# Luka140/paig_reproduction

Measured on AMD Instinct MI355X. Metric: video-seqs/sec (train step) spring_color B=100 @ 1/2/4/8 MI355X, higher is better.
Workload: dtype fp32; 1 GPU; spring_color PhysicsNet train step (get_batch gather+fwd+loss+bwd+allreduce+RMSprop), B=100/rank, 32x32x3, seq_len 50 (4 in / 6 pred / 40 extrap); global_batch=100, seq_len=50, parallelism=dp1, conv_math=split, split_graph=False, optimizer_in_graph=True, byte_targets=True, dataset_seqs=800

## Files before the change

### paig_reproduction_amd/csrc/conv_bwd.hip

```cpp
#include "split_common.h"

#include <stdlib.h>

#ifndef PAIG_BWD_MINW
#define PAIG_BWD_MINW 0
#endif
#ifndef PAIG_BWD_UPS2
#define PAIG_BWD_UPS2 1
#endif
#ifndef PAIG_BWD_TPX_C10
#define PAIG_BWD_TPX_C10 0
#define PAIG_BWD_MINW_C10 0
#endif
#ifndef PAIG_BWD_PSD_EVEN_C10
#define PAIG_BWD_PSD_EVEN_C10 0
#endif
#ifndef PAIG_BWD_AUXP
#define PAIG_BWD_AUXP 1
#endif

#ifdef PAIG_BWD_STAMPS
__device__ unsigned long long paig_bwd_stamps[4096][4][13];
#define PAIG_BSTAMP(k)                                      \
  do {                                                      \
// ... 9 lines not shown

namespace {

constexpr int sbwd_lds(int CIN, int COUT, int H, int W, bool UPS, int PM, int tpx) {
  const int FPT = H * W <= tpx ? tpx / (H * W) : 1, RT = H * W <= tpx ? H : rows_fit(H, W, tpx);
  const bool pe = PAIG_BWD_PSD_EVEN_C10 && UPS && CIN == 16 && COUT == 16 && H == 32;
  const int ROWS = RT + 2, ROWSD = ROWS + (UPS ? 2 : 0), CCD = rup(COUT, 8) / 8,
            PSD = CCD % 2 == 0 && !pe ? CCD + 1 : CCD;
  const int RPD = W == 8 ? to_mod16((W + 2) * PSD, 8) : (W + 2) * PSD;
  const int IMGD = (FPT * ROWSD * RPD + 2) * 8, WIMG = ceil_div(9 * CCD, 4) * ceil_div(CIN, 16) * 64 * 8;
  const int XIMG = rup(CIN, 4) / 4 * rup(FPT * ROWS * (W + 4) * 4 + 80, 128) * 2 * (PM == 2 ? 1 : 2);
  const int UPB = UPS ? CIN * (rup(FPT * (RT + 2) * W, 64) + 4) * 4 : 0;
  const int XREG = XIMG > UPB ? XIMG : UPB;
  return (IMGD + WIMG) * 2 * (PM == 2 ? 1 : 2) + XREG + (UPS ? up_window_floats(CIN, FPT, RT, W) * 4 : 0);
}
constexpr int sbwd_tpx(int CIN, int COUT, int H, int W, bool UPS, int PM) {
  if (PAIG_BWD_TPX_C10 && UPS && CIN == 16 && COUT == 16 && H == 32) return PAIG_BWD_TPX_C10;
  for (int pass = 0; pass < 2; ++pass)
    for (int t = 256; t >= 64; t /= 2) {
      const int rt = H * W <= t ? H : rows_fit(H, W, t);
      if (UPS && (rt % 2 != 0 || H * W < t)) continue;
      if (sbwd_lds(CIN, COUT, H, W, UPS, PM, t) <= (pass == 0 ? LDS_MAX / 2 : LDS_MAX)) return t;
    }
  return 64;
}

constexpr int sbwd_minw(int CIN, int COUT, int H, int PM, bool PF) {
  if (PAIG_BWD_MINW_C10 && CIN == 16 && COUT == 16 && H == 32) return PAIG_BWD_MINW_C10;
  if (CIN == 8 && COUT == 8 && H == 32) return PF || PAIG_BWD_AUXP == 2 ? 3 : 4;
  if (PM == 2 && CIN == 8 && COUT == 16 && H == 16) return 3;
  if (PM == 2 && CIN == 24 && COUT == 8 && H == 32) return 3;
  if (CIN == 8 && COUT == 8 && H == 36) return PF ? 2 : 3;
  if (CIN == 8 && COUT == 16 && H == 18) return PM == 2 ? 4 : 3;
  if (CIN == 16 && COUT == 16 && H == 18) return PF ? 2 : 3;
  return 2;
}

constexpr bool sbwd_auxp(int CIN, int COUT, int H, int PM, bool UPS, bool PF) {
  if (PAIG_BWD_AUXP == 2) return true;
  if (CIN == 8 && COUT == 8 && (H == 32 || H == 36) && !PF) return false;
  if (CIN == 24 && COUT == 8 && (H == 36 || PM == 2)) return false;
  if (UPS && H == 36) return false;
  if (PM == 0) return !(PF && CIN == 16 && COUT == 16 && H == 16);
  return !((UPS && CIN == 32 && H == 16) || (CIN == 8 && COUT == 16 && H == 16));
}

template <int CIN, int COUT, int H, int W, int KS, bool UPS, int PM, bool PF = false>
struct SBwdCfg {
  static constexpr int KK = KS * KS, PADL = KS / 2;
  static constexpr int NIMG = PM == 2 ? 1 : 2;
  static constexpr int TPX = sbwd_tpx(CIN, COUT, H, W, UPS, PM);
  static constexpr int FPT = H * W <= TPX ? TPX / (H * W) : 1;
  static constexpr int RT = H * W <= TPX ? H : rows_fit(H, W, TPX);
  static constexpr int TPXV = FPT * RT * W;
  static constexpr int ROWS = RT + KS - 1;
  static constexpr int EXT = UPS ? 1 : 0;
  static constexpr int RTD = RT + 2 * EXT, ROWSD = ROWS + 2 * EXT;
  static constexpr int TPXD = FPT * RTD * W;
  static constexpr int CCD = rup(COUT, 8) / 8;
  static constexpr bool PSDE = PAIG_BWD_PSD_EVEN_C10 && UPS && CIN == 16 && COUT == 16 && H == 32;
  static constexpr int PSD = CCD % 2 == 0 && !PSDE ? CCD + 1 : CCD;
  static constexpr int TWPX = W + 2 * PADL;
  static constexpr int RPD = W == 8 ? to_mod16(TWPX * PSD, 8) : TWPX * PSD;
  static constexpr int ZSLOT = FPT * ROWSD * RPD;
  static constexpr int IMGD = (ZSLOT + 2) * 8;
  static constexpr int KC = KK * CCD, NS = ceil_div(KC, 4);
  static constexpr int NTD = ceil_div(CIN, 16);
  static constexpr int NMT = ceil_div(TPXD, 16), MW = ceil_div(NMT, 4);
  static constexpr int WIMG = NS * NTD * 64 * 8;
  static constexpr int CQ = rup(CIN, 4) / 4, NQ = KK * CQ, NTX = ceil_div(NQ, 4);
  static constexpr int OFFX = PADL > 0 ? 2 : 0, TWX = W + 2 * OFFX;
  static constexpr int XPL = rup(FPT * ROWS * TWX * 4 + 80, 128);
  static constexpr int XIMG = CQ * XPL;
  static constexpr int MT = ceil_div(COUT, 16), NTW = ceil_div(NTX, 4);
  static constexpr bool BAL = !(PM == 2 && (CIN == 24 || (UPS && CIN == 32) || H == 36 || H == 18)) && !(H == 36 && !UPS && !PF);
  static constexpr int NTF = BAL ? NTX / 4 : ceil_div(NTX, 4), NTR = BAL ? NTX % 4 : 0;
  static constexpr int KB = ceil_div(TPXV, 32);
  static constexpr int NCOL = CIN * KK, SLAB = COUT * NCOL + COUT;
  static constexpr int UPX = W % 2 == 0 ? 2 : 1, W2 = W / UPX;
  static constexpr int NID = FPT * ROWSD * W2 * CCD, NLD = ceil_div(NID, 256);
  static constexpr int NIX = FPT * ROWS * W2 * CQ, NLX = ceil_div(NIX, 256);
  static constexpr int UPW = up_window_floats(CIN, FPT, RT, W);
  static constexpr int UPB = UPS ? CIN * (rup(FPT * (RT + 2) * W, 64) + 4) * 4 : 0;
  static constexpr int XREG = XIMG * 2 * NIMG > UPB ? XIMG * 2 * NIMG : UPB;
  static constexpr int LDS = (IMGD + WIMG) * 2 * NIMG + XREG + (UPS ? UPW * 4 : 0);
  static constexpr bool VEC4 = W % 4 == 0;
  static constexpr bool XPIPE = !UPS && NLX * 8 <= 32;
  static constexpr int LDSB = LDS_MAX / (LDS > (NLD * 256 * 8 + 256) * 4 ? LDS : (NLD * 256 * 8 + 256) * 4);
  static constexpr int MW0 = PAIG_BWD_MINW > 0 ? PAIG_BWD_MINW : sbwd_minw(CIN, COUT, H, PM, PF);
  static constexpr int MINW = MW0 < LDSB ? MW0 : LDSB;
  static_assert(H % RT == 0, "RT divides H");
  static_assert(KS == 3, "3x3 layers (the 1x1 heads are fused elsewhere)");
  static_assert(!UPS || (FPT == 1 && RT % 2 == 0 && W % 2 == 0), "fused upsample: whole even row blocks of one frame");
  static_assert(!PF || (!UPS && UPX == 2 && COUT % 8 == 0 && H % 2 == 0), "pool fold: even widths, 8-channel chunks");
  static constexpr int UPP = rup(TPXD, 64) + 4;
  static_assert(!UPS || CIN * UPP * 4 <= XREG, "fused upsample: dX tile does not fit the X region");
  static constexpr int WSU = W / 2, IKU = WSU % 4 == 0 ? 4 : (WSU % 2 == 0 ? 2 : 1), WQU = WSU / IKU;
  static constexpr int NOU = UPS ? CIN * (RT / 2) * WQU : 0, NOI = NOU > 0 ? ceil_div(NOU, 256) : 1;
  static constexpr bool AUXP =
      PAIG_BWD_AUXP && (UPS || (VEC4 && MW * NTD <= 8)) && sbwd_auxp(CIN, COUT, H, PM, UPS, PF);
};

template <int CIN, int COUT, int H, int W, int KS, bool UPS, int PM, bool PF>
__global__ void __launch_bounds__(256, (SBwdCfg<CIN, COUT, H, W, KS, UPS, PM, PF>::MINW))
conv_bwd_split_k(FView x, FView dy, FViewW dx, FView aux, const float* __restrict__ w, int flags,
                 float* __restrict__ slab, int F, int ntiles, XMax xm, const s16x8* __restrict__ wp, FView dpool,
                 const unsigned char* __restrict__ pcode, long long pcode_fs) {
  using C = SBwdCfg<CIN, COUT, H, W, KS, UPS, PM, PF>;
  constexpr int KK = C::KK, PADL = C::PADL, RT = C::RT, FPT = C::FPT, ROWS = C::ROWS, TPXV = C::TPXV;
  constexpr int EXT = C::EXT, RTD = C::RTD, ROWSD = C::ROWSD, TPXD = C::TPXD;
  constexpr int CCD = C::CCD, PSD = C::PSD, RPD = C::RPD, KC = C::KC, NS = C::NS, NTD = C::NTD, MW = C::MW;
  constexpr int CQ = C::CQ, NQ = C::NQ, NTX = C::NTX, OFFX = C::OFFX, TWX = C::TWX, XPL = C::XPL;
  constexpr int MT = C::MT, NTF = C::NTF, NTR = C::NTR, KB = C::KB, NCOL = C::NCOL, UPX = C::UPX, W2 = C::W2;
  constexpr int NF1 = NTF > 0 ? NTF : 1, NR1 = NTR > 0 ? NTR : 1;
  constexpr int NID = C::NID, NLD = C::NLD, NIX = C::NIX, NLX = C::NLX;
  constexpr long long HW = (long long)H * W;
  constexpr long long XPLANE = UPS ? (long long)(H / 2) * (W / 2) : HW;
  constexpr int NRB = H / RT;
  extern __shared__ __attribute__((aligned(16))) short lds16[];
  short* Dh = lds16;
  short* Dl = Dh + (C::NIMG == 2 ? C::IMGD : 0);
  short* Wh = lds16 + C::NIMG * C::IMGD;
  short* Wl = Wh + (C::NIMG == 2 ? C::WIMG : 0);
  short* Xh = lds16 + C::NIMG * (C::IMGD + C::WIMG);
  short* Xl = Xh + (C::NIMG == 2 ? C::XIMG : 0);
// ... 122 lines not shown
  for (int t = 0; t < NTR; ++t) coltr[t] = colt_of(NTF * 4 + t);
  auto dslot = [&](int j) {
    if (TPXV % 32 != 0 && j >= TPXV) return C::ZSLOT;
    const int fi = j / (RT * W), rem = j % (RT * W);
    return (fi * ROWSD + rem / W + PADL + EXT) * RPD + (rem % W + PADL) * PSD;
  };
  auto xpos = [&](int j) {
    if (TPXV % 32 != 0 && j >= TPXV) j = 0;
    const int fi = j / (RT * W), rem = j % (RT * W);
    return ((fi * ROWS + rem / W) * TWX + rem % W + (OFFX - PADL)) * 4;
  };

  f32x4 accw[MT][NF1], accr[MT][NR1];
#pragma unroll
  for (int m = 0; m < MT; ++m) {
#pragma unroll
    for (int j = 0; j < NF1; ++j) accw[m][j] = f32x4{0.f, 0.f, 0.f, 0.f};
#pragma unroll
    for (int t = 0; t < NR1; ++t) accr[m][t] = f32x4{0.f, 0.f, 0.f, 0.f};
  }
  float bacc[NLD][8];
#pragma unroll
  for (int l = 0; l < NLD; ++l)
#pragma unroll
    for (int c = 0; c < 8; ++c) bacc[l][c] = 0.f;

  float2 pd[NLD][8];
  float2 px[C::XPIPE ? NLX : 1][4];
  float dpv[PF ? NLD : 1][8];
  uint2 pcv[PF ? NLD : 1];
  constexpr int HP = H / 2, WP = W / 2;
  using UP = UpStage<UPS ? CIN : 1, H, W, FPT, RT>;
  UP up;
  auto load_d = [&](int t) {
    const int f0 = (t / NRB) * FPT, y0 = (t % NRB) * RT;
    const float* fb = dy.frame(f0 < F ? f0 : 0);
#pragma unroll
    for (int l = 0; l < NLD; ++l) {
      const int i = tid + l * 256;
      const int xp = UPX * (i % W2), r = (i / W2) % ROWSD, cc = (i / (W2 * ROWSD)) % CCD, fi = i / (W2 * ROWSD * CCD);
      const int gy = y0 + r - PADL - EXT;
#ifdef PAIG_BWD_NOLOAD
      const bool ok = false;
#else
      const bool ok = i < NID && f0 + fi < F && gy >= 0 && gy < H;
#endif
      const int off = fi * (int)dy.fs + cc * 8 * (int)HW + gy * W + xp;
      static_assert(8 * HW <= 8 * 4096, "paig_zero_planes covers the unit");
      const float* base = ok ? fb + off : paig_zero_planes;
#pragma unroll
      for (int c = 0; c < 8; ++c) {
        const float* q = COUT % 8 == 0 || cc * 8 + c < COUT ? base + c * (int)HW : paig_zeros;
        pd[l][c] = UPX == 2 ? *reinterpret_cast<const float2*>(q) : make_float2(*q, 0.f);
      }
      if constexpr (PF) {
        const int pw = (gy >> 1) * WP + (xp >> 1);
        const float* pb = ok ? dpool.frame(f0) + fi * (int)dpool.fs + cc * 8 * (HP * WP) + pw : paig_zero_planes;
#pragma unroll
        for (int c = 0; c < 8; ++c) dpv[l][c] = pb[c * (HP * WP)];
        const unsigned char* cb = ok ? pcode + (long long)(f0 + fi) * pcode_fs + ((long long)cc * HP * WP + pw) * 8
                                     : reinterpret_cast<const unsigned char*>(paig_zeros);
        pcv[l] = *reinterpret_cast<const uint2*>(cb);
      }
    }
  };
  auto fold = [&](int t) {
    const int y0 = (t % NRB) * RT;
#pragma unroll
    for (int l = 0; l < NLD; ++l) {
      const int i = tid + l * 256;
      const int r = (i / W2) % ROWSD;
      const int pr = ((y0 + r - PADL - EXT) & 1) * 2;
#pragma unroll
      for (int c = 0; c < 8; ++c) {
        const unsigned b = ((c < 4 ? pcv[l].x : pcv[l].y) >> (8 * (c & 3))) & 255u;
        const int am = (int)(b >> 4) & 3;
        const float vx = pd[l][c].x + (am == pr ? dpv[l][c] : 0.f);
        const float vy = pd[l][c].y + (am == pr + 1 ? dpv[l][c] : 0.f);
        pd[l][c].x = (b >> pr) & 1u ? vx : 0.f;
        pd[l][c].y = (b >> (pr + 1)) & 1u ? vy : 0.f;
      }
    }
  };
  auto load_x = [&](int t, int i, float2* v) {
    const int f0 = (t / NRB) * FPT, y0 = (t % NRB) * RT;
    const int xp = UPX * (i % W2), r = (i / W2) % ROWS, cq = (i / (W2 * ROWS)) % CQ, fi = i / (W2 * ROWS * CQ);
    const int gy = y0 + r - PADL;
    const bool ok = i < NIX && f0 + fi < F && gy >= 0 && gy < H;
    const float* fb = x.frame(f0 < F ? f0 : 0);
    const int off = fi * (int)x.fs + cq * 4 * (int)XPLANE + gy * W + xp;
    const float* base = ok ? fb + off : paig_zero_planes;
#pragma unroll
    for (int c = 0; c < 4; ++c) {
      const float* q = CIN % 4 == 0 || cq * 4 + c < CIN ? base + c * (int)XPLANE : paig_zeros;
      v[c] = UPX == 2 ? *reinterpret_cast<const float2*>(q) : make_float2(*q, 0.f);
    }
  };
  auto issue = [&](int t) {
    load_d(t);
    if constexpr (UPS) {
      up.issue(x, F, (t / NRB) * FPT, (t % NRB) * RT, tid);
    } else if constexpr (C::XPIPE) {
#pragma unroll
      for (int l = 0; l < NLX; ++l) load_x(t, tid + l * 256, px[l]);
    }
  };
  auto put_d = [&](int i, const float2* v) {
    const int xp = UPX * (i % W2), r = (i / W2) % ROWSD, cc = (i / (W2 * ROWSD)) % CCD, fi = i / (W2 * ROWSD * CCD);
    const int o = ((fi * ROWSD + r) * RPD + (xp + PADL) * PSD + cc) * 8;
    s16x8 h0, l0, h1, l1;
    if constexpr (PM == 0) {
      pf32x2 sv[8];
#pragma unroll
      for (int c = 0; c < 8; ++c) sv[c] = pf32x2{v[c].x, v[c].y} * dsc;
      u32x4 a0, b0, a1, b1;
#pragma unroll
      for (int k = 0; k < 4; ++k) {
        { const HiLo q_ = split_pk(sv[2 * k].x, sv[2 * k + 1].x); a0[k] = q_.h; b0[k] = q_.l; }
        { const HiLo q_ = split_pk(sv[2 * k].y, sv[2 * k + 1].y); a1[k] = q_.h; b1[k] = q_.l; }
      }
      h0 = __builtin_bit_cast(s16x8, a0);
      l0 = __builtin_bit_cast(s16x8, b0);
      h1 = __builtin_bit_cast(s16x8, a1);
      l1 = __builtin_bit_cast(s16x8, b1);
    } else {
      float rm = 0.f;
#pragma unroll
      for (int c = 0; c < 8; ++c) {
        short h, lo;
        split<PM>(v[c].x, h, lo, rm);
        h0[c] = h;
        l0[c] = lo;
        split<PM>(v[c].y, h, lo, rm);
        h1[c] = h;
        l1[c] = lo;
      }
    }
    *reinterpret_cast<s16x8*>(Dh + o) = h0;
    if (PM != 2) *reinterpret_cast<s16x8*>(Dl + o) = l0;
    if constexpr (UPX == 2) {
      *reinterpret_cast<s16x8*>(Dh + o + PSD * 8) = h1;
      if (PM != 2) *reinterpret_cast<s16x8*>(Dl + o + PSD * 8) = l1;
    }
  };
  auto put_x = [&](int i, const float2* v) {
    const int xp = UPX * (i % W2), r = (i / W2) % ROWS, cq = (i / (W2 * ROWS)) % CQ, fi = i / (W2 * ROWS * CQ);
    const int o = xplane(cq) + ((fi * ROWS + r) * TWX + xp + OFFX) * 4;
    s16x8 hv, lv;
    if constexpr (PM == 0) {
      pf32x2 sv[4];
#pragma unroll
      for (int c = 0; c < 4; ++c) {
        sv[c] = pf32x2{v[c].x, v[c].y} * xsc;
        rmax = amax2(rmax, sv[c].x, sv[c].y);
      }
      u32x4 a, b;
      { const HiLo q_ = split_pk(sv[0].x, sv[1].x); a[0] = q_.h; b[0] = q_.l; }
      { const HiLo q_ = split_pk(sv[2].x, sv[3].x); a[1] = q_.h; b[1] = q_.l; }
      { const HiLo q_ = split_pk(sv[0].y, sv[1].y); a[2] = q_.h; b[2] = q_.l; }
      { const HiLo q_ = split_pk(sv[2].y, sv[3].y); a[3] = q_.h; b[3] = q_.l; }
      hv = __builtin_bit_cast(s16x8, a);
      lv = __builtin_bit_cast(s16x8, b);
    } else {
#pragma unroll
      for (int c = 0; c < 4; ++c) {
        short h, lo;
        split<PM>(v[c].x, h, lo, rmax);
        hv[c] = h;
        lv[c] = lo;
        split<PM>(v[c].y, h, lo, rmax);
        hv[4 + c] = h;
        lv[4 + c] = lo;
      }
    }
    if constexpr (UPX == 2) {
      *reinterpret_cast<s16x8*>(Xh + o) = hv;
      if (PM != 2) *reinterpret_cast<s16x8*>(Xl + o) = lv;
    } else {
      *reinterpret_cast<s16x4*>(Xh + o) = s16x4{hv[0], hv[1], hv[2], hv[3]};
      if (PM != 2) *reinterpret_cast<s16x4*>(Xl + o) = s16x4{lv[0], lv[1], lv[2], lv[3]};
    }
  };
  auto tile_max = [&]() {
    float m = 0.f;
#pragma unroll
    for (int l = 0; l < NLD; ++l)
#pragma unroll
      for (int c = 0; c < 8; ++c) m = amax2(m, pd[l][c].x, pd[l][c].y);
    m = wave_max_u(m);
    if (lane == 0) smax[wv] = m;
  };
  auto commit = [&](int t) {
    if constexpr (PM == 0 && PAIG_SCALE_MODE < 2) {
      const int te = f16_scale_exp(fmaxf(fmaxf(smax[0], smax[1]), fmaxf(smax[2], smax[3])));
      const int td = te < ecd + 64 ? te : ecd + 64;
      if (td != ecd) {
#pragma unroll
        for (int m = 0; m < MT; ++m)
#pragma unroll
          for (int r = 0; r < 4; ++r) {
#pragma unroll
            for (int j = 0; j < NF1; ++j) accw[m][j][r] = __builtin_amdgcn_ldexpf(accw[m][j][r], td - ecd);
#pragma unroll
            for (int t = 0; t < NR1; ++t) accr[m][t][r] = __builtin_amdgcn_ldexpf(accr[m][t][r], td - ecd);
          }
        ecd = td;
        dsc = __builtin_amdgcn_ldexpf(1.f, ecd);
      }
    }
    const int f0 = (t / NRB) * FPT;
#pragma unroll
    for (int l = 0; l < NLD; ++l) {
      const int i = tid + l * 256;
      if (NID % 256 != 0 && i >= NID) break;
      put_d(i, pd[l]);
      const int r = (i / W2) % ROWSD, fi = i / (W2 * ROWSD * CCD);
      if (r >= PADL + EXT && r < PADL + EXT + RT && f0 + fi < F) {
#pragma unroll
        for (int c = 0; c < 8; ++c) bacc[l][c] += pd[l][c].x + pd[l][c].y;
      }
    }
    PAIG_BSTAMP(8);
    if constexpr (UPS) {
      const int y0 = (t % NRB) * RT;
      up.commit(Sl, tid);
      zero_xhalo();
      PAIG_BSTAMP(9);
      __syncthreads();
      PAIG_BSTAMP(10);
      if constexpr (W % 4 == 0 && ROWS % 2 == 0 && PAIG_BWD_UPS2 && PM == 0 && H != 36) {
        constexpr int W4 = W / 4, RP2 = ROWS / 2;
#pragma unroll 1
        for (int i = tid; i < CQ * RP2 * W4; i += 256) {
          const int q = i % W4, rp = (i / W4) % RP2, cq = i / (W4 * RP2);
          const int gy = y0 + 2 * rp - PADL;
          const bool ok0 = f0 < F && gy >= 0 && gy < H, ok1 = f0 < F && gy + 1 >= 0 && gy + 1 < H;
          f32x4 o0[4], o1[4];
#pragma unroll
          for (int c = 0; c < 4; ++c) {
            if (cq * 4 + c < CIN) {
              UP::row4x2(Sl, 0, cq * 4 + c, gy, y0, q, ok0, ok1, o0[c], o1[c]);
            } else {
              o0[c] = f32x4{0.f, 0.f, 0.f, 0.f};
              o1[c] = o0[c];
            }
          }
#pragma unroll
          for (int h2 = 0; h2 < 2; ++h2) {
            const int ia = (cq * ROWS + 2 * rp + h2) * W2 + 2 * q;
            const f32x4* o = h2 ? o1 : o0;
// ... 21 lines not shown
#pragma unroll
          for (int c = 0; c < 4; ++c)
            o[c] = (ok && cq * 4 + c < CIN) ? UP::row4(Sl, 0, cq * 4 + c, gy, y0, q) : f32x4{0.f, 0.f, 0.f, 0.f};
          const int ia = (cq * ROWS + r) * W2 + 2 * q;
          float2 v[4];
#pragma unroll
          for (int c = 0; c < 4; ++c) v[c] = make_float2(o[c][0], o[c][1]);
          put_x(ia, v);
#pragma unroll
          for (int c = 0; c < 4; ++c) v[c] = make_float2(o[c][2], o[c][3]);
          put_x(ia + 1, v);
        }
        PAIG_BSTAMP(11);
      } else {
#pragma unroll 1
        for (int i = tid; i < NIX; i += 256) {
          const int xp = UPX * (i % W2), r = (i / W2) % ROWS, cq = (i / (W2 * ROWS)) % CQ;
          const int gy = y0 + r - PADL;
          const bool ok = f0 < F && gy >= 0 && gy < H;
          float2 v[4];
#pragma unroll
          for (int c = 0; c < 4; ++c)
            v[c] = (ok && cq * 4 + c < CIN)
                       ? make_float2(UP::px1(Sl, 0, cq * 4 + c, gy, y0, xp), UP::px1(Sl, 0, cq * 4 + c, gy, y0, xp + 1))
                       : make_float2(0.f, 0.f);
          put_x(i, v);
        }
      }
    } else if constexpr (C::XPIPE) {
#pragma unroll
      for (int l = 0; l < NLX; ++l) {
        const int i = tid + l * 256;
        if (NIX % 256 != 0 && i >= NIX) break;
        put_x(i, px[l]);
      }
    } else {
#pragma unroll 1
      for (int i = tid; i < NIX; i += 256) {
        float2 v[4];
        load_x(t, i, v);
        put_x(i, v);
      }
    }
  };

  int lt = blockIdx.x;
  auto tile_of = [&](int l) { return l < ntiles ? xcd_tile(l, ntiles) : ntiles; };
  issue(tile_of(lt));
  if (PM == 0 && xm.p) {
    float m = 0.f;
    for (int i = tid * 4; i < xm.n; i += 1024) {
      const f32x4 v = *reinterpret_cast<const f32x4*>(xm.p + i);
      m = fmaxf(m, fmaxf(fmaxf(v[0], v[1]), fmaxf(v[2], v[3])));
    }
    m = wave_max_u(m);
    if (lane == 0) smax[wv] = m;
    __syncthreads();
    m = fmaxf(fmaxf(smax[0], smax[1]), fmaxf(smax[2], smax[3]));
    if (m > 0.f) ecx = f16_scale_exp(m);
    __syncthreads();
  }
  if constexpr (PM == 0) xsc = __builtin_amdgcn_ldexpf(1.f, ecx);
  else ecx = 0;

  PAIG_BSTAMP(0);
  for (; lt < ntiles; lt += gridDim.x) {
    const int tile = xcd_tile(lt, ntiles);
    const int f0 = (tile / NRB) * FPT, y0 = (tile % NRB) * RT;
    if constexpr (PF) fold(tile);
    if constexpr (PM == 0 && PAIG_SCALE_MODE < 2) tile_max();
    __syncthreads();
    PAIG_BSTAMP(1);
    commit(tile);
    __syncthreads();
    PAIG_BSTAMP(2);
    typedef float fIKU __attribute__((ext_vector_type(C::IKU)));
    f32x4 auxv[C::AUXP && !UPS ? MW : 1][C::AUXP && !UPS ? NTD : 1];
    fIKU auxu[C::AUXP && UPS ? C::NOI : 1];
    if constexpr (C::AUXP) {
      if (flags & 2) {
        if constexpr (UPS) {
#pragma unroll
          for (int k = 0; k < C::NOI; ++k) {
            const int o = tid + 256 * k;
            const int q = o % C::WQU, sr = (o / C::WQU) % (RT / 2), ci = o / (C::WQU * (RT / 2));
            const bool ok = o < C::NOU && f0 < F;
            const float* ap = ok ? aux.frame(f0) + ((long long)ci * (H / 2) + y0 / 2 + sr) * C::WSU + C::IKU * q
                                 : paig_zero_planes;
            auxu[k] = *reinterpret_cast<const fIKU*>(ap);
          }
        } else {
#pragma unroll
          for (int nt = 0; nt < NTD; ++nt) {
            const int ci = nt * 16 + (lane & 15);
#pragma unroll
            for (int mt = 0; mt < MW; ++mt) {
              const int pix = (wv * MW + mt) * 16 + (lane >> 4) * 4;
              const int fi = pix / (RT * W), rem = pix % (RT * W);
              const int f = f0 + fi;
              const bool ok = ci < CIN && pix < TPXV && f < F;
              const float* ap = ok ? aux.frame(f) + ci * HW + (long long)(y0 + rem / W) * W + rem % W
                                   : paig_zero_planes;
              auxv[mt][nt] = *reinterpret_cast<const f32x4*>(ap);
            }
          }
        }
      }
    }
    issue(tile_of(lt + gridDim.x));
    PAIG_BSTAMP(3);

#pragma unroll 2
    for (int kb = 0; kb < KB; ++kb) {
      const int p0 = kb * 32;
      s16x8 ah[MT], al[MT];
      const int d0 = dslot(p0 + 8 * g + qq), d1 = dslot(p0 + 8 * g + 4 + qq);
#pragma unroll
      for (int m = 0; m < MT; ++m) {
        const int co = 2 * m + (pl >> 1), hoff = (pl & 1) * 4;
        const int a0 = (d0 + co) * 8 + hoff, a1 = (d1 + co) * 8 + hoff;
        ah[m] = __builtin_shufflevector(tr_read(Dh + a0), tr_read(Dh + a1), 0, 1, 2, 3, 4, 5, 6, 7);
        al[m] = PM != 2 ? __builtin_shufflevector(tr_read(Dl + a0), tr_read(Dl + a1), 0, 1, 2, 3, 4, 5, 6, 7) : ah[m];
      }
      const int r0 = xpos(p0 + 8 * g + qq), r1 = xpos(p0 + 8 * g + 4 + qq);
      auto ntile = [&](int ct, f32x4* acc) __attribute__((always_inline)) {
        const s16x8 bh = __builtin_shufflevector(tr_read(Xh + r0 + ct), tr_read(Xh + r1 + ct), 0, 1, 2, 3, 4, 5, 6, 7);
        const s16x8 bl =
            PM != 2 ? __builtin_shufflevector(tr_read(Xl + r0 + ct), tr_read(Xl + r1 + ct), 0, 1, 2, 3, 4, 5, 6, 7) : bh;
#pragma unroll
        for (int m = 0; m < MT; ++m) acc[m] = mma3<PM>(ah[m], al[m], bh, bl, acc[m]);
      };
#pragma unroll
      for (int jn = 0; jn < NTF; ++jn) {
        if (!C::BAL && wv + jn * 4 >= NTX) continue;
        f32x4 a[MT];
#pragma unroll
        for (int m = 0; m < MT; ++m) a[m] = accw[m][jn];
// ... 251 lines not shown
                       FView dpool = FView{nullptr, 0, 0, 0}, const unsigned char* pcode = nullptr,
                       long long pcode_fs = 0) {
  using C = SBwdCfg<CIN, COUT, H, W, KS, UPS, PM, PF>;
  constexpr int RED = (C::NLD * 256 * 8 + 256) * 4;
  constexpr int LDS0 = C::LDS > RED ? C::LDS : RED;
  static_assert(LDS0 <= LDS_MAX, "fused backward: staging exceeds the LDS");
  static const int lds_pad = [] {
    const char* e = getenv("PAIG_BWD_LDS_PAD");
    return e ? atoi(e) : 0;
  }();
  const int LDS = LDS0 + lds_pad <= LDS_MAX ? LDS0 + lds_pad : LDS0;
  const int ntiles = cdiv(F, C::FPT) * (H / C::RT);
  auto k = conv_bwd_split_k<CIN, COUT, H, W, KS, UPS, PM, PF>;
  static int resident = 0;
  if (!resident) {
    if (LDS > 64 * 1024) (void)hipFuncSetAttribute((const void*)k, hipFuncAttributeMaxDynamicSharedMemorySize, LDS);
    resident = persistent_grid((const void*)k, LDS);
  }
  int nb = ntiles < nblk_max ? ntiles : nblk_max;
  if (nb > resident) nb = resident;
  {
    static int mt = -1;
    if (mt < 0) {
      const char* e = getenv("PAIG_BWD_MIN_TPB");
      mt = e ? atoi(e) : 0;
    }
    if (mt > 1 && nb > cdiv(ntiles, mt)) nb = cdiv(ntiles, mt);
  }
  if (nb < 1) nb = 1;
  *nblk_out = nb;
  PAIG_REQUIRE(!xm.p || (xm.n % 4 == 0 && (reinterpret_cast<uintptr_t>(xm.p) & 15) == 0),
               "conv split bwd: xmax needs 16-byte alignment and a multiple of 4 slots (%d)", xm.n);
  PAIG_REQUIRE(!(flags & 2) || aux.p, "conv split bwd: ReLU' mask (flags & 2) without aux");
  PAIG_REQUIRE(!PF || (dpool.p && pcode && (reinterpret_cast<uintptr_t>(pcode) & 7) == 0 && pcode_fs % 8 == 0),
               "conv split bwd: pool fold needs the pooled gradient and 8-byte aligned window codes");
  hipLaunchKernelGGL(k, dim3(nb), dim3(256), LDS, st, x, dy, dx, aux, w, flags, slab, F, ntiles, xm,
                     PM == 0 ? static_cast<const s16x8*>(wp) : nullptr, dpool, pcode, pcode_fs);
  PAIG_CHECK_LAUNCH();
  return 0;
}

#define PAIG_BWD_UP_SHAPES(X) X(32, 16, 16) X(16, 16, 32) X(16, 16, 36) X(32, 16, 18)
#define PAIG_BWD_POOL_SHAPES(X) X(8, 8, 32) X(16, 16, 16) X(16, 16, 64) X(8, 8, 36) X(16, 16, 18)
#define PAIG_BWD_SHAPES(X)                                                                  \
  X(8, 8, 32) X(8, 16, 16) X(16, 16, 16) X(16, 32, 8) X(32, 32, 8) X(32, 16, 16) X(24, 8, 32) \
  X(8, 8, 36) X(8, 16, 18) X(16, 16, 18) X(32, 16, 18) X(24, 8, 36)                            \
  X(16, 16, 64) X(16, 32, 32)

}

extern "C" {

int paig_conv2d_bwd_supported(int Cin, int Cout, int H, int W, int ks, int flags) {
  if (H != W || ks != 3 || !(flags & (128 | 256))) return 0;
#define PAIG_CASE(CI, CO, HH) \
  if (Cin == CI && Cout == CO && H == HH) return 1;
  if (flags & 64) {
    if (flags & 32) return 0;
    PAIG_BWD_POOL_SHAPES(PAIG_CASE)
    return 0;
  }
  if (flags & 32) {
    PAIG_BWD_UP_SHAPES(PAIG_CASE)
    return 0;
  }
  PAIG_BWD_SHAPES(PAIG_CASE)
// ... 66 lines not shown
```

### paig_reproduction_amd/csrc/split_common.h

```cpp
#pragma once
#include "conv_tile.h"

#ifndef PAIG_SCALE_MODE
#define PAIG_SCALE_MODE 0
#endif

namespace {

typedef short s16x8 __attribute__((ext_vector_type(8)));
typedef short s16x4 __attribute__((ext_vector_type(4)));
typedef __bf16 bf16x8 __attribute__((ext_vector_type(8)));
typedef _Float16 f16x8 __attribute__((ext_vector_type(8)));
typedef __attribute__((address_space(3))) s16x4 lds_s16x4;
typedef unsigned u32x4 __attribute__((ext_vector_type(4)));
typedef unsigned u32x2 __attribute__((ext_vector_type(2)));

constexpr int rup(int a, int b) { return ceil_div(a, b) * b; }

__device__ __forceinline__ int xcd_tile(int L, int ntiles) {
  return (ntiles % 8 == 0 && gridDim.x % 8 == 0) ? (L % 8) * (ntiles / 8) + L / 8 : L;
}
constexpr int rows_fit(int n, int w, int cap) {
  int best = 1;
  for (int d = 1; d <= n; ++d)
// ... 15 lines not shown
    h = __builtin_bit_cast(short, a);
    if constexpr (PM == 1) {
      const __bf16 b = (__bf16)(v - (float)a);
      l = __builtin_bit_cast(short, b);
    } else {
      l = 0;
    }
  }
}

template <int PM>
__device__ __forceinline__ f32x4 mma(s16x8 a, s16x8 b, f32x4 c) {
  if constexpr (PM == 0)
    return __builtin_amdgcn_mfma_f32_16x16x32_f16(__builtin_bit_cast(f16x8, a), __builtin_bit_cast(f16x8, b), c, 0,
                                                  0, 0);
  else
    return __builtin_amdgcn_mfma_f32_16x16x32_bf16(__builtin_bit_cast(bf16x8, a), __builtin_bit_cast(bf16x8, b), c,
                                                   0, 0, 0);
}

template <int PM>
__device__ __forceinline__ f32x4 mma3(s16x8 ah, s16x8 al, s16x8 bh, s16x8 bl, f32x4 c) {
  if constexpr (PM != 2) {
    c = mma<PM>(al, bh, c);
    c = mma<PM>(ah, bl, c);
  }
  return mma<PM>(ah, bh, c);
}

__device__ __forceinline__ s16x4 tr_read(const short* p) {
  return __builtin_amdgcn_ds_read_tr16_b64_v4i16((lds_s16x4*)p);
}

#ifndef PAIG_UPS_CPAD
#define PAIG_UPS_CPAD 0
#endif
constexpr int up_pitch(int RT, int W) { return (RT / 2 + 2 + (RT & 1)) * (W / 2) + PAIG_UPS_CPAD; }
constexpr int up_window_floats(int CIN, int FPT, int RT, int W) { return FPT * CIN * up_pitch(RT, W); }

template <int CIN, int H, int W, int FPT, int RT>
struct UpStage {
  static constexpr int HS = H / 2, WS = W / 2, SRN = RT / 2 + 2 + (RT & 1);
  static constexpr int VS = WS % 4 == 0 ? 4 : 1;
  static constexpr int QS = WS / VS;
  static constexpr int NSU = FPT * CIN * SRN * QS, NLS = (NSU + 255) / 256;
  static constexpr int CP = up_pitch(RT, W);
  static constexpr int SL = up_window_floats(CIN, FPT, RT, W);
  f32x4 v[VS == 4 ? NLS : 1];
  float v1[VS == 1 ? NLS : 1];
  __device__ __forceinline__ void issue(const FView& x, int F, int f0, int y0, int tid) {
#pragma unroll
    for (int l = 0; l < NLS; ++l) {
      const int i = tid + l * 256;
      const int q = i % QS, sr = (i / QS) % SRN, c = (i / (QS * SRN)) % CIN, fi = i / (QS * SRN * CIN);
      const int srow = y0 / 2 - 1 + sr;
      const bool ok = i < NSU && f0 + fi < F && srow >= 0 && srow < HS;
      const float* src = ok ? x.frame(f0) + fi * (int)x.fs + c * HS * WS + srow * WS + VS * q : paig_zeros;
      if constexpr (VS == 4) v[l] = *reinterpret_cast<const f32x4*>(src);
      else v1[l] = *src;
    }
  }
  __device__ __forceinline__ float amax() const {
    float m = 0.f;
#pragma unroll
    for (int l = 0; l < NLS; ++l) {
      if constexpr (VS == 4) m = amax2(amax2(m, v[l][0], v[l][1]), v[l][2], v[l][3]);
      else m = fmaxf(m, fabsf(v1[l]));
    }
    return m;
  }
  __device__ __forceinline__ void commit(float* Sl, int tid) const {
#pragma unroll
    for (int l = 0; l < NLS; ++l) {
      const int i = tid + l * 256;
      if (NSU % 256 != 0 && i >= NSU) break;
      const int fc = i / (QS * SRN), r = i % (QS * SRN);
      if constexpr (VS == 4) *reinterpret_cast<f32x4*>(Sl + fc * CP + 4 * r) = v[l];
      else Sl[fc * CP + r] = v1[l];
    }
  }
  static __device__ __forceinline__ float px1(const float* Sl, int fi, int c, int gy, int y0, int x) {
    int ya, yb, xa, xb;
    float wa, wb, ua, ub;
    up2_taps(gy, HS, ya, yb, wa, wb);
    up2_taps(x, WS, xa, xb, ua, ub);
    const float* p = Sl + (fi * CIN + c) * CP;
    const float* r0 = p + (ya - (y0 / 2 - 1)) * WS;
    const float* r1 = p + (yb - (y0 / 2 - 1)) * WS;
    return wa * (ua * r0[xa] + ub * r0[xb]) + wb * (ua * r1[xa] + ub * r1[xb]);
  }
  static __device__ __forceinline__ f32x4 row4(const float* Sl, int fi, int c, int gy, int y0, int q) {
    int ya, yb;
// ... 51 lines not shown
```

Baseline: 99050 video-seqs/s.

## Switch conv backward global loads to buffer loads with hoisted per-thread offsets

Replaces pointer-based global loads of dY, X, pooled gradient, window codes and ReLU aux in the split conv backward kernel with AMD raw buffer loads. Out-of-bounds lanes now get zeros from the buffer descriptor's range check instead of being redirected to a zero page. Per-thread index decomposition (div/mod chains) is precomputed once outside the tile loop for most layer configs, gated by a new per-shape HOIST table. One occupancy hint is also adjusted. The aim is fewer integer ALU ops and 64-bit address computations per tile, at the cost of extra registers for the hoisted offsets and a new 32-bit offset range requirement on frame strides.

```diff
diff --git a/paig_reproduction_amd/csrc/conv_bwd.hip b/paig_reproduction_amd/csrc/conv_bwd.hip
--- a/paig_reproduction_amd/csrc/conv_bwd.hip
+++ b/paig_reproduction_amd/csrc/conv_bwd.hip
@@ -65,7 +65,7 @@
   if (PM == 2 && CIN == 24 && COUT == 8 && H == 32) return 3;
   if (CIN == 8 && COUT == 8 && H == 36) return PF ? 2 : 3;
   if (CIN == 8 && COUT == 16 && H == 18) return PM == 2 ? 4 : 3;
-  if (CIN == 16 && COUT == 16 && H == 18) return PF ? 2 : 3;
+  if (CIN == 16 && COUT == 16 && H == 18) return PF && PM != 2 ? 2 : 3;
   return 2;
 }
 
@@ -76,6 +76,14 @@
   if (UPS && H == 36) return false;
   if (PM == 0) return !(PF && CIN == 16 && COUT == 16 && H == 16);
   return !((UPS && CIN == 32 && H == 16) || (CIN == 8 && COUT == 16 && H == 16));
+}
+
+constexpr bool sbwd_hoist(int CIN, int COUT, int H, int PM, bool PF) {
+  if (PF && PM == 0 && ((CIN == 8 && H == 32) || H == 64)) return false;
+  if (PF && PM == 2 && H == 18) return false;
+  if (CIN == 24 && H == 36 && PM == 0) return false;
+  if (H == 18 && ((CIN == 8 && PM == 2) || (CIN == 16 && COUT == 16 && PM == 0))) return false;
+  return true;
 }
 
 template <int CIN, int COUT, int H, int W, int KS, bool UPS, int PM, bool PF = false>
@@ -118,12 +126,14 @@
   static constexpr int XREG = XIMG * 2 * NIMG > UPB ? XIMG * 2 * NIMG : UPB;
   static constexpr int LDS = (IMGD + WIMG) * 2 * NIMG + XREG + (UPS ? UPW * 4 : 0);
   static constexpr bool VEC4 = W % 4 == 0;
+  static constexpr bool HOIST = sbwd_hoist(CIN, COUT, H, PM, PF);
   static constexpr bool XPIPE = !UPS && NLX * 8 <= 32;
   static constexpr int LDSB = LDS_MAX / (LDS > (NLD * 256 * 8 + 256) * 4 ? LDS : (NLD * 256 * 8 + 256) * 4);
   static constexpr int MW0 = PAIG_BWD_MINW > 0 ? PAIG_BWD_MINW : sbwd_minw(CIN, COUT, H, PM, PF);
   static constexpr int MINW = MW0 < LDSB ? MW0 : LDSB;
   static_assert(H % RT == 0, "RT divides H");
   static_assert(KS == 3, "3x3 layers (the 1x1 heads are fused elsewhere)");
+  static_assert(COUT % 8 == 0 && CIN % 4 == 0, "staging units of 8 dY / 4 X channels");
   static_assert(!UPS || (FPT == 1 && RT % 2 == 0 && W % 2 == 0), "fused upsample: whole even row blocks of one frame");
   static_assert(!PF || (!UPS && UPX == 2 && COUT % 8 == 0 && H % 2 == 0), "pool fold: even widths, 8-channel chunks");
   static constexpr int UPP = rup(TPXD, 64) + 4;
@@ -312,35 +322,101 @@
   constexpr int HP = H / 2, WP = W / 2;
   using UP = UpStage<UPS ? CIN : 1, H, W, FPT, RT>;
   UP up;
+  auto row_ok = [&](int gy) { return (unsigned)gy < (unsigned)H; };
+  auto d_unit = [&](int i, int& vo, int& row, int& so) {
+    const int xp = UPX * (i % W2), r = (i / W2) % ROWSD, cc = (i / (W2 * ROWSD)) % CCD, fi = i / (W2 * ROWSD * CCD);
+#ifdef PAIG_BWD_NOLOAD
+    const bool in = false;
+#else
+    const bool in = i < NID;
+#endif
+    row = in ? r - PADL - EXT : -(1 << 20);
+    vo = (fi * (int)dy.fs + cc * 8 * (int)HW + (r - PADL - EXT) * W + xp) * 4;
+    if (NRB == 1 && !row_ok(row)) vo = BUF_OOR;
+    so = ((fi * ROWSD + r) * RPD + (xp + PADL) * PSD + cc) * 8;
+  };
+  constexpr int NLH = C::HOIST ? NLD : 1;
+  int dvo[NLH], drow[NLH], dso[NLH];
+  if constexpr (C::HOIST) {
+#pragma unroll
+    for (int l = 0; l < NLD; ++l) d_unit(tid + l * 256, dvo[l], drow[l], dso[l]);
+  }
+  auto d_get = [&](int l, int& vo, int& row, int& so) {
+    if constexpr (C::HOIST) {
+      vo = dvo[l];
+      row = drow[l];
+      so = dso[l];
+    } else {
+      d_unit(opaque(tid) + l * 256, vo, row, so);
+    }
+  };
+  auto pf_unit = [&](int i, int& po, int& co) {
+    const int xp = UPX * (i % W2), cc = (i / (W2 * ROWSD)) % CCD, fi = i / (W2 * ROWSD * CCD);
+    po = (fi * (int)dpool.fs + cc * 8 * (HP * WP) + (xp >> 1)) * 4;
+    co = fi * (int)pcode_fs + (cc * (HP * WP) + (xp >> 1)) * 8;
+  };
+  auto x_unit = [&](int i, int& vo, int& row, int& so) {
+    const int xp = UPX * (i % W2), r = (i / W2) % ROWS, cq = (i / (W2 * ROWS)) % CQ, fi = i / (W2 * ROWS * CQ);
+    row = i < NIX ? r - PADL : -(1 << 20);
+    vo = (fi * (int)x.fs + cq * 4 * (int)XPLANE + (r - PADL) * W + xp) * 4;
+    if (NRB == 1 && !row_ok(row)) vo = BUF_OOR;
+    so = xplane(cq) + ((fi * ROWS + r) * TWX + xp + OFFX) * 4;
+  };
+  constexpr int NXH = C::XPIPE && C::HOIST ? NLX : 1;
+  int xvo[NXH], xrow[NXH], xso[NXH];
+  if constexpr (C::XPIPE && C::HOIST) {
+#pragma unroll
+    for (int l = 0; l < NLX; ++l) x_unit(tid + l * 256, xvo[l], xrow[l], xso[l]);
+  }
+  auto x_get = [&](int l, int& vo, int& row, int& so) {
+    if constexpr (C::HOIST) {
+      vo = xvo[l];
+      row = xrow[l];
+      so = xso[l];
+    } else {
+      x_unit(opaque(tid) + l * 256, vo, row, so);
+    }
+  };
+  int uvo[UPS ? UP::NLS : 1], urow[UPS ? UP::NLS : 1];
+  if constexpr (UPS) {
+#pragma unroll
+    for (int l = 0; l < UP::NLS; ++l) UP::unit(tid + l * 256, (int)x.fs, uvo[l], urow[l]);
+  }
+  auto tile_nf = [&](int f0) {
+    const int n = F - f0;
+    return n < FPT ? n : FPT;
+  };
+  auto tile_vo = [&](int vo, int row, int y0) {
+    if constexpr (NRB == 1) return vo;
+    else return row_ok(y0 + row) ? vo + y0 * W * 4 : BUF_OOR;
+  };
   auto load_d = [&](int t) {
-    const int f0 = (t / NRB) * FPT, y0 = (t % NRB) * RT;
-    const float* fb = dy.frame(f0 < F ? f0 : 0);
+    const int f0 = (t / NRB) * FPT, y0 = (t % NRB) * RT, nf = tile_nf(f0);
+    const brsrc rd = tile_rsrc(dy.frame(f0), dy.fs, nf, COUT * (int)HW);
+    brsrc rp, rc;
+    if constexpr (PF) {
+      rp = tile_rsrc(dpool.frame(f0), dpool.fs, nf, COUT * HP * WP);
+      rc = tile_rsrc(pcode + (long long)f0 * pcode_fs, pcode_fs, nf, CCD * HP * WP * 8, 1);
+    }
 #pragma unroll
     for (int l = 0; l < NLD; ++l) {
-      const int i = tid + l * 256;
-      const int xp = UPX * (i % W2), r = (i / W2) % ROWSD, cc = (i / (W2 * ROWSD)) % CCD, fi = i / (W2 * ROWSD * CCD);
-      const int gy = y0 + r - PADL - EXT;
-#ifdef PAIG_BWD_NOLOAD
-      const bool ok = false;
-#else
-      const bool ok = i < NID && f0 + fi < F && gy >= 0 && gy < H;
-#endif
-      const int off = fi * (int)dy.fs + cc * 8 * (int)HW + gy * W + xp;
-      static_assert(8 * HW <= 8 * 4096, "paig_zero_planes covers the unit");
-      const float* base = ok ? fb + off : paig_zero_planes;
+      int vo0, row, so;
+      d_get(l, vo0, row, so);
+      const int vo = tile_vo(vo0, row, y0);
 #pragma unroll
       for (int c = 0; c < 8; ++c) {
-        const float* q = COUT % 8 == 0 || cc * 8 + c < COUT ? base + c * (int)HW : paig_zeros;
-        pd[l][c] = UPX == 2 ? *reinterpret_cast<const float2*>(q) : make_float2(*q, 0.f);
+        pd[l][c] = UPX == 2 ? buf_ld2(rd, vo, c * (int)HW * 4) : make_float2(buf_ld1(rd, vo, c * (int)HW * 4), 0.f);
       }
       if constexpr (PF) {
-        const int pw = (gy >> 1) * WP + (xp >> 1);
-        const float* pb = ok ? dpool.frame(f0) + fi * (int)dpool.fs + cc * 8 * (HP * WP) + pw : paig_zero_planes;
-#pragma unroll
-        for (int c = 0; c < 8; ++c) dpv[l][c] = pb[c * (HP * WP)];
-        const unsigned char* cb = ok ? pcode + (long long)(f0 + fi) * pcode_fs + ((long long)cc * HP * WP + pw) * 8
-                                     : reinterpret_cast<const unsigned char*>(paig_zeros);
-        pcv[l] = *reinterpret_cast<const uint2*>(cb);
+        const int wr = ((y0 + row) >> 1) * WP;
+        const bool ok = NRB == 1 ? vo != BUF_OOR : row_ok(y0 + row);
+        int po, co;
+        pf_unit(opaque(tid) + l * 256, po, co);
+        const int vp = ok ? po + wr * 4 : BUF_OOR;
+#pragma unroll
+        for (int c = 0; c < 8; ++c) dpv[l][c] = buf_ld1(rp, vp, c * (HP * WP) * 4);
+        const u32x2 cv = __builtin_amdgcn_raw_buffer_load_b64(rc, ok ? co + wr * 8 : BUF_OOR, 0, 0);
+        pcv[l] = make_uint2(cv.x, cv.y);
       }
     }
   };
@@ -348,9 +424,9 @@
     const int y0 = (t % NRB) * RT;
 #pragma unroll
     for (int l = 0; l < NLD; ++l) {
-      const int i = tid + l * 256;
-      const int r = (i / W2) % ROWSD;
-      const int pr = ((y0 + r - PADL - EXT) & 1) * 2;
+      int vo, row, so;
+      d_get(l, vo, row, so);
+      const int pr = ((y0 + row) & 1) * 2;
 #pragma unroll
       for (int c = 0; c < 8; ++c) {
         const unsigned b = ((c < 4 ? pcv[l].x : pcv[l].y) >> (8 * (c & 3))) & 255u;
@@ -362,32 +438,32 @@
       }
     }
   };
-  auto load_x = [&](int t, int i, float2* v) {
-    const int f0 = (t / NRB) * FPT, y0 = (t % NRB) * RT;
-    const int xp = UPX * (i % W2), r = (i / W2) % ROWS, cq = (i / (W2 * ROWS)) % CQ, fi = i / (W2 * ROWS * CQ);
-    const int gy = y0 + r - PADL;
-    const bool ok = i < NIX && f0 + fi < F && gy >= 0 && gy < H;
-    const float* fb = x.frame(f0 < F ? f0 : 0);
-    const int off = fi * (int)x.fs + cq * 4 * (int)XPLANE + gy * W + xp;
-    const float* base = ok ? fb + off : paig_zero_planes;
-#pragma unroll
-    for (int c = 0; c < 4; ++c) {
-      const float* q = CIN % 4 == 0 || cq * 4 + c < CIN ? base + c * (int)XPLANE : paig_zeros;
-      v[c] = UPX == 2 ? *reinterpret_cast<const float2*>(q) : make_float2(*q, 0.f);
-    }
+  auto x_rsrc = [&](int t) {
+    const int f0 = (t / NRB) * FPT;
+    return tile_rsrc(x.frame(f0), x.fs, tile_nf(f0), CIN * (int)XPLANE);
+  };
+  auto load_x = [&](brsrc rx, int t, int vo0, int row, float2* v) {
+    const int vo = tile_vo(vo0, row, (t % NRB) * RT);
+#pragma unroll
+    for (int c = 0; c < 4; ++c)
+      v[c] = UPX == 2 ? buf_ld2(rx, vo, c * (int)XPLANE * 4) : make_float2(buf_ld1(rx, vo, c * (int)XPLANE * 4), 0.f);
   };
   auto issue = [&](int t) {
+    if (t >= ntiles) return;
     load_d(t);
     if constexpr (UPS) {
-      up.issue(x, F, (t / NRB) * FPT, (t % NRB) * RT, tid);
+      up.issue(x_rsrc(t), (t % NRB) * RT, uvo, urow);
     } else if constexpr (C::XPIPE) {
-#pragma unroll
-      for (int l = 0; l < NLX; ++l) load_x(t, tid + l * 256, px[l]);
-    }
-  };
-  auto put_d = [&](int i, const float2* v) {
-    const int xp = UPX * (i % W2), r = (i / W2) % ROWSD, cc = (i / (W2 * ROWSD)) % CCD, fi = i / (W2 * ROWSD * CCD);
-    const int o = ((fi * ROWSD + r) * RPD + (xp + PADL) * PSD + cc) * 8;
+      const brsrc rx = x_rsrc(t);
+#pragma unroll
+      for (int l = 0; l < NLX; ++l) {
+        int vo, row, so;
+        x_get(l, vo, row, so);
+        load_x(rx, t, vo, row, px[l]);
+      }
+    }
+  };
+  auto put_d = [&](int o, const float2* v) {
     s16x8 h0, l0, h1, l1;
     if constexpr (PM == 0) {
       pf32x2 sv[8];
@@ -423,9 +499,7 @@
       if (PM != 2) *reinterpret_cast<s16x8*>(Dl + o + PSD * 8) = l1;
     }
   };
-  auto put_x = [&](int i, const float2* v) {
-    const int xp = UPX * (i % W2), r = (i / W2) % ROWS, cq = (i / (W2 * ROWS)) % CQ, fi = i / (W2 * ROWS * CQ);
-    const int o = xplane(cq) + ((fi * ROWS + r) * TWX + xp + OFFX) * 4;
+  auto put_x_at = [&](int o, const float2* v) {
     s16x8 hv, lv;
     if constexpr (PM == 0) {
       pf32x2 sv[4];
@@ -461,6 +535,10 @@
       if (PM != 2) *reinterpret_cast<s16x4*>(Xl + o) = s16x4{lv[0], lv[1], lv[2], lv[3]};
     }
   };
+  auto put_x = [&](int i, const float2* v) {
+    const int xp = UPX * (i % W2), r = (i / W2) % ROWS, cq = (i / (W2 * ROWS)) % CQ, fi = i / (W2 * ROWS * CQ);
+    put_x_at(xplane(cq) + ((fi * ROWS + r) * TWX + xp + OFFX) * 4, v);
+  };
   auto tile_max = [&]() {
     float m = 0.f;
 #pragma unroll
@@ -493,9 +571,10 @@
     for (int l = 0; l < NLD; ++l) {
       const int i = tid + l * 256;
       if (NID % 256 != 0 && i >= NID) break;
-      put_d(i, pd[l]);
-      const int r = (i / W2) % ROWSD, fi = i / (W2 * ROWSD * CCD);
-      if (r >= PADL + EXT && r < PADL + EXT + RT && f0 + fi < F) {
+      int vo, row, so;
+      d_get(l, vo, row, so);
+      put_d(so, pd[l]);
+      if ((unsigned)row < (unsigned)RT) {
 #pragma unroll
         for (int c = 0; c < 8; ++c) bacc[l][c] += pd[l][c].x + pd[l][c].y;
       }
@@ -583,20 +662,42 @@
       for (int l = 0; l < NLX; ++l) {
         const int i = tid + l * 256;
         if (NIX % 256 != 0 && i >= NIX) break;
-        put_x(i, px[l]);
+        int vo, row, so;
+        x_get(l, vo, row, so);
+        put_x_at(so, px[l]);
       }
     } else {
+      const brsrc rx = x_rsrc(t);
 #pragma unroll 1
       for (int i = tid; i < NIX; i += 256) {
         float2 v[4];
-        load_x(t, i, v);
-        put_x(i, v);
-      }
-    }
-  };
+        int vo, row, so;
+        x_unit(i, vo, row, so);
+        load_x(rx, t, vo, row, v);
+        put_x_at(so, v);
+      }
+    }
+  };
+
+  int avo[C::AUXP ? (UPS ? C::NOI : MW) : 1];
+  if constexpr (C::AUXP && UPS) {
+#pragma unroll
+    for (int k = 0; k < C::NOI; ++k) {
+      const int o = tid + 256 * k;
+      const int q = o % C::WQU, sr = (o / C::WQU) % (RT / 2), ci = o / (C::WQU * (RT / 2));
+      avo[k] = o < C::NOU ? ((ci * (H / 2) + sr) * C::WSU + C::IKU * q) * 4 : BUF_OOR;
+    }
+  } else if constexpr (C::AUXP) {
+#pragma unroll
+    for (int mt = 0; mt < MW; ++mt) {
+      const int pix = (wv * MW + mt) * 16 + (lane >> 4) * 4;
+      const int fi = pix / (RT * W), rem = pix % (RT * W);
+      avo[mt] = pix < TPXV ? (fi * (int)aux.fs + (lane & 15) * (int)HW + rem) * 4 : BUF_OOR;
+    }
+  }
 
   int lt = blockIdx.x;
-  auto tile_of = [&](int l) { return l < ntiles ? xcd_tile(l, ntiles) : ntiles; };
+  auto tile_of =[&](int l) { return l < ntiles ? xcd_tile(l, ntiles) : ntiles; };
   issue(tile_of(lt));
   if (PM == 0 && xm.p) {
     float m = 0.f;
@@ -630,30 +731,22 @@
     fIKU auxu[C::AUXP && UPS ? C::NOI : 1];
     if constexpr (C::AUXP) {
       if (flags & 2) {
+        const brsrc ra = tile_rsrc(aux.frame(f0), aux.fs, tile_nf(f0), CIN * (int)XPLANE);
         if constexpr (UPS) {
 #pragma unroll
           for (int k = 0; k < C::NOI; ++k) {
-            const int o = tid + 256 * k;
-            const int q = o % C::WQU, sr = (o / C::WQU) % (RT / 2), ci = o / (C::WQU * (RT / 2));
-            const bool ok = o < C::NOU && f0 < F;
-            const float* ap = ok ? aux.frame(f0) + ((long long)ci * (H / 2) + y0 / 2 + sr) * C::WSU + C::IKU * q
-                                 : paig_zero_planes;
-            auxu[k] = *reinterpret_cast<const fIKU*>(ap);
+            const int so = (y0 / 2) * C::WSU * 4;
+            if constexpr (C::IKU == 4) auxu[k] = buf_ld4(ra, avo[k], so);
+            else if constexpr (C::IKU == 2) auxu[k] = __builtin_bit_cast(fIKU, buf_ld2(ra, avo[k], so));
+            else auxu[k] = __builtin_bit_cast(fIKU, buf_ld1(ra, avo[k], so));
           }
         } else {
 #pragma unroll
           for (int nt = 0; nt < NTD; ++nt) {
-            const int ci = nt * 16 + (lane & 15);
-#pragma unroll
-            for (int mt = 0; mt < MW; ++mt) {
-              const int pix = (wv * MW + mt) * 16 + (lane >> 4) * 4;
-              const int fi = pix / (RT * W), rem = pix % (RT * W);
-              const int f = f0 + fi;
-              const bool ok = ci < CIN && pix < TPXV && f < F;
-              const float* ap = ok ? aux.frame(f) + ci * HW + (long long)(y0 + rem / W) * W + rem % W
-                                   : paig_zero_planes;
-              auxv[mt][nt] = *reinterpret_cast<const f32x4*>(ap);
-            }
+            const bool cok = CIN % 16 == 0 || nt * 16 + (lane & 15) < CIN;
+#pragma unroll
+            for (int mt = 0; mt < MW; ++mt)
+              auxv[mt][nt] = buf_ld4(ra, cok ? avo[mt] : BUF_OOR, (nt * 16 * (int)HW + y0 * W) * 4);
           }
         }
       }
@@ -971,6 +1064,10 @@
   PAIG_REQUIRE(!xm.p || (xm.n % 4 == 0 && (reinterpret_cast<uintptr_t>(xm.p) & 15) == 0),
                "conv split bwd: xmax needs 16-byte alignment and a multiple of 4 slots (%d)", xm.n);
   PAIG_REQUIRE(!(flags & 2) || aux.p, "conv split bwd: ReLU' mask (flags & 2) without aux");
+  constexpr long long SPAN = (1ll << 31) / (4 * C::FPT) - 8 * 4096;
+  PAIG_REQUIRE(x.fs < SPAN && dy.fs < SPAN && aux.fs < SPAN && dpool.fs < SPAN && pcode_fs < 4 * SPAN &&
+                   x.fs >= 0 && dy.fs >= 0 && aux.fs >= 0 && dpool.fs >= 0 && pcode_fs >= 0,
+               "conv split bwd: a frame stride does not fit the tile's 32-bit byte offsets");
   PAIG_REQUIRE(!PF || (dpool.p && pcode && (reinterpret_cast<uintptr_t>(pcode) & 7) == 0 && pcode_fs % 8 == 0),
                "conv split bwd: pool fold needs the pooled gradient and 8-byte aligned window codes");
   hipLaunchKernelGGL(k, dim3(nb), dim3(256), LDS, st, x, dy, dx, aux, w, flags, slab, F, ntiles, xm,
diff --git a/paig_reproduction_amd/csrc/split_common.h b/paig_reproduction_amd/csrc/split_common.h
--- a/paig_reproduction_amd/csrc/split_common.h
+++ b/paig_reproduction_amd/csrc/split_common.h
@@ -71,6 +71,25 @@
   return __builtin_amdgcn_ds_read_tr16_b64_v4i16((lds_s16x4*)p);
 }
 
+typedef __amdgpu_buffer_rsrc_t brsrc;
+constexpr int BUF_OOR = (int)0x80000000u;
+__device__ __forceinline__ brsrc buf_rsrc(const void* p, int bytes) {
+  return __builtin_amdgcn_make_buffer_rsrc(const_cast<void*>(p), 0, bytes, 0x00020000);
+}
+__device__ __forceinline__ brsrc tile_rsrc(const void* frame0, long long fs, int nf, int cf, int esz = 4) {
+  return buf_rsrc(frame0, nf > 0 ? ((nf - 1) * (int)fs + cf) * esz : 0);
+}
+__device__ __forceinline__ float buf_ld1(brsrc r, int vo, int s) {
+  return __builtin_bit_cast(float, __builtin_amdgcn_raw_buffer_load_b32(r, vo, s, 0));
+}
+__device__ __forceinline__ float2 buf_ld2(brsrc r, int vo, int s) {
+  const pf32x2 v = __builtin_bit_cast(pf32x2, __builtin_amdgcn_raw_buffer_load_b64(r, vo, s, 0));
+  return make_float2(v.x, v.y);
+}
+__device__ __forceinline__ f32x4 buf_ld4(brsrc r, int vo, int s) {
+  return __builtin_bit_cast(f32x4, __builtin_amdgcn_raw_buffer_load_b128(r, vo, s, 0));
+}
+
 #ifndef PAIG_UPS_CPAD
 #define PAIG_UPS_CPAD 0
 #endif
@@ -97,6 +116,20 @@
       const float* src = ok ? x.frame(f0) + fi * (int)x.fs + c * HS * WS + srow * WS + VS * q : paig_zeros;
       if constexpr (VS == 4) v[l] = *reinterpret_cast<const f32x4*>(src);
       else v1[l] = *src;
+    }
+  }
+  static __device__ __forceinline__ void unit(int i, int fs, int& uo, int& ur) {
+    const int q = i % QS, sr = (i / QS) % SRN, c = (i / (QS * SRN)) % CIN, fi = i / (QS * SRN * CIN);
+    ur = i < NSU ? sr - 1 : -(1 << 20);
+    uo = (fi * fs + c * HS * WS + (sr - 1) * WS + VS * q) * 4;
+  }
+  __device__ __forceinline__ void issue(brsrc r, int y0, const int* uo, const int* ur) {
+    const int ro = (y0 / 2) * WS * 4;
+#pragma unroll
+    for (int l = 0; l < NLS; ++l) {
+      const int vo = (unsigned)(y0 / 2 + ur[l]) < (unsigned)HS ? uo[l] + ro : BUF_OOR;
+      if constexpr (VS == 4) v[l] = buf_ld4(r, vo, 0);
+      else v1[l] = buf_ld1(r, vo, 0);
     }
   }
   __device__ __forceinline__ float amax() const {
```

Measured after the change: 100,100 video-seqs/s, median of 6. 1.01x the previous value.
